# clysto/tinyimgcodec

Hardware: AMD Instinct MI355X
Metric: Mpixels/s encode (DCT+quant kernel) (higher is better)
Workload: dtype f32+f64

## Files before the change

tinyimgcodec_amd/csrc/tic_kernels.hip:

```cpp
#include <hip/hip_runtime.h>
#include <hip/hip_ext.h>
#include <stdint.h>
#include <stdlib.h>
#include <string.h>
#include <type_traits>

#include "tic_hooks.h"
#include "tic_kernels.h"
#include "tic_math.h"

namespace tic {

#define TIC_DPP_QP_XOR1 0xB1
#define TIC_DPP_QP_XOR2 0x4E
#define TIC_DPP_ROW_SHL4 0x104
#define TIC_DPP_ROW_SHR4 0x114

__device__ __forceinline__ uint32_t perm_b32(uint32_t hi_src, uint32_t lo_src, uint32_t sel) {
    return __builtin_amdgcn_perm(hi_src, lo_src, sel);
}

__device__ __forceinline__ void transpose8x8_bytes(uint32_t &lo, uint32_t &hi, int i) {
    uint32_t nhi = (uint32_t)__builtin_amdgcn_update_dpp((int)hi, (int)lo, TIC_DPP_ROW_SHL4, 0xf, 0x5, false);
    uint32_t nlo = (uint32_t)__builtin_amdgcn_update_dpp((int)lo, (int)hi, TIC_DPP_ROW_SHR4, 0xf, 0xa, false);
// ... 148 lines not shown
    const int lane = threadIdx.x & 63, wave = threadIdx.x >> 6;
    const int b = lane >> 3, i = lane & 7;
    uint32_t *lds = lds_all[wave];
    int tile = blockIdx.x * kWavesPerWG + wave;
    int ntiles = a.ntiles;
    if (a.rem_mode) {
        const int bh = a.ntiles / a.tiles_x, rw = a.tiles_x - a.fast_tx;
        const int n_right = bh * rw, n_bottom = (bh - a.fast_ty) * a.fast_tx;
        ntiles = 0;
        if (tile < n_right) {
            tile = (tile / rw) * a.tiles_x + a.fast_tx + tile % rw;
            ntiles = a.ntiles;
        } else if (tile < n_right + n_bottom) {
            const int k = tile - n_right;
            tile = (a.fast_ty + k / a.fast_tx) * a.tiles_x + k % a.fast_tx;
            ntiles = a.ntiles;
        }
    }
    Strip s = make_strip(tile, ntiles, a.tiles_x, a.bw, b);
    uint32_t lo, hi;
    load_block_row(a.img, a.h, a.w, a.stride, a.aligned8, s, i, lo, hi);
    transpose8x8_bytes(lo, hi, i);
    int q[8];
    exact_block(lo, hi, lds, b, i, a.consts, q);
    const uint4 zzv = *reinterpret_cast<const uint4 *>(a.consts->zzofs + i * 8);
    uint16_t zz[8] = {(uint16_t)zzv.x, (uint16_t)(zzv.x >> 16), (uint16_t)zzv.y, (uint16_t)(zzv.y >> 16),
                      (uint16_t)zzv.z, (uint16_t)(zzv.z >> 16), (uint16_t)zzv.w, (uint16_t)(zzv.w >> 16)};
    store_zigzag(lds, b, i, zz, q, a.out, s);
}

constexpr int kTWaveBytes = kLdsWaveBytes;
constexpr int kTHalfDw = 272;
constexpr int kZzWaveBytes = 8 * kZzStrideB;
constexpr int kPxBlkBytes = 80;
constexpr int kMaxStripsPerWave = 16;
constexpr int kChunkStrips = 8;

__device__ __forceinline__ void quant_fma(float z, float mul, uint32_t &bits, float &d) {
    const float s = fmaf(z, mul, kMagic);
    bits = __float_as_uint(s);
    const float nr = kMagic - s;
    d = fmaf(z, mul, nr);
}

__device__ __forceinline__ void store16_wt_nt(void *p, const uint4 &v) {
    typedef uint32_t u32x4 __attribute__((ext_vector_type(4)));
    const u32x4 d = {v.x, v.y, v.z, v.w};
    asm volatile("global_store_dwordx4 %0, %1, off sc1 nt" : : "v"(p), "v"(d) : "memory");
}
__device__ __forceinline__ void store16_wt_nt(const void *sbase, uint32_t voff, const uint4 &v) {
    typedef uint32_t u32x4 __attribute__((ext_vector_type(4)));
    const u32x4 d = {v.x, v.y, v.z, v.w};
    asm volatile("global_store_dwordx4 %0, %1, %2 sc1 nt" : : "v"(voff), "v"(d), "s"(sbase) : "memory");
}

constexpr int kMaxStripsPerWave2 = 64;
constexpr int kBatch = 8;
constexpr int kBatchWaveBytes = kBatch * (128 + 64) + 64;

template <int CTRL>
__device__ __forceinline__ double dpp_f64(double x) {
    const int lo = __builtin_amdgcn_mov_dpp(__double2loint(x), CTRL, 0xf, 0xf, true);
    const int hi = __builtin_amdgcn_mov_dpp(__double2hiint(x), CTRL, 0xf, 0xf, true);
    return __hiloint2double(hi, lo);
}

__device__ __forceinline__ int rational_quad(const uint32_t *ldsT, int b, int i, const double *cst_rat) {
#pragma clang fp contract(off)
    const int w = i >> 2, k = i & 3;
    const uint32_t ca = (0x05010300u >> (8 * k)) & 0xffu, cb = (0x06020407u >> (8 * k)) & 0xffu;
    const uint32_t *row = ldsT + w * 128 + 4 * b;
    const float fa = __uint_as_float(row[(ca >> 2) * kTHalfDw + (ca & 3)]);
    const float fb = __uint_as_float(row[(cb >> 2) * kTHalfDw + (cb & 3)]);
    const double K = w ? (kTW3 * 0.5) : (kSq2h * 0.5);
    const double ya = (double)fa * K, yb = (double)fb * K;
    const double p = ya + yb;
    const double s2 = p + dpp_f64<TIC_DPP_QP_XOR1>(p);
    const double o = dpp_f64<TIC_DPP_QP_XOR2>(s2);
    const double E = (k & 1) ? s2 - o : s2 + o;
    const double X = E * ((k & 1) ? (kTW3 * 0.5) : (kSq2h * 0.5));
    const double div = cst_rat[2 * w + (k & 1)], rdiv = cst_rat[4 + 2 * w + (k & 1)];
    return (int)rint(div_rn(X, div, rdiv));
}

__device__ __forceinline__ int rational_slim(uint32_t rowLo, uint32_t rowHi, int i, const double *cst_rat) {
#pragma clang fp contract(off)
    uint32_t lo = perm_b32(rowHi, rowLo, 0x04030700u);
    uint32_t hi = perm_b32(rowHi, rowLo, 0x06050201u);
    transpose8x8_bytes(lo, hi, i);
    const uint32_t tot = __builtin_amdgcn_sad_u8(lo, 0u, __builtin_amdgcn_sad_u8(hi, 0u, 0u));
    const uint32_t sa = __builtin_amdgcn_sad_u8(lo & 0xff0000ffu, 0u, __builtin_amdgcn_sad_u8(hi & 0xff0000ffu, 0u, 0u));
    const int e0 = (int)tot - 1024, e4 = 2 * (int)sa - (int)tot;
    double y0 = (double)e0 * (kSq2h * 0.5);
    double y4 = (double)e4 * (kTW3 * 0.5);
    y0 = y0 + dpp_f64<TIC_DPP_QP_XOR1>(y0);
    y4 = y4 + dpp_f64<TIC_DPP_QP_XOR1>(y4);
    y0 = y0 + dpp_f64<TIC_DPP_QP_XOR2>(y0);
    y4 = y4 + dpp_f64<TIC_DPP_QP_XOR2>(y4);
    const double b0 = dpp_f64<TIC_DPP_ROW_SHL4>(y0), b4 = dpp_f64<TIC_DPP_ROW_SHL4>(y4);
    const double A = (i & 2) ? y4 : y0, B = (i & 2) ? b4 : b0;
    const double E = (i & 1) ? A - B : A + B;
    const double X = E * ((i & 1) ? (kTW3 * 0.5) : (kSq2h * 0.5));
    const double div = cst_rat[i & 3], rdiv = cst_rat[4 + (i & 3)];
    return (int)rint(div_rn(X, div, rdiv));
}
__device__ __forceinline__ unsigned long long wave_redo_block(const uint8_t *px , double *tbuf ,
                                                              const double *cosm, const double *rdiv, const uint16_t *zzofs, int16_t *img16,
                                                              int lane) {
    const int u = lane >> 3, c = lane & 7;
    typedef double d2 __attribute__((ext_vector_type(2)));
    const d2 *mu = reinterpret_cast<const d2 *>(cosm + u * 8), *mc = reinterpret_cast<const d2 *>(cosm + c * 8);
    const d2 m0 = mu[0], m1 = mu[1], m2 = mu[2], m3 = mu[3];
    double x[8];
#pragma unroll
    for (int r = 0; r < 8; r++) x[r] = (double)((int)px[r * 8 + c] - 128);
    double ta = m0.x * x[0], tb = m0.y * x[1];
    ta = fma(m1.x, x[2], ta); tb = fma(m1.y, x[3], tb);
    ta = fma(m2.x, x[4], ta); tb = fma(m2.y, x[5], tb);
    ta = fma(m3.x, x[6], ta); tb = fma(m3.y, x[7], tb);
    tbuf[u * 8 + c] = ta + tb;
    const d2 n0 = mc[0], n1 = mc[1], n2 = mc[2], n3 = mc[3];
    wave_lds_fence();
    const d2 *tu = reinterpret_cast<const d2 *>(tbuf + u * 8);
    const d2 y0 = tu[0], y1 = tu[1], y2 = tu[2], y3 = tu[3];
    double xa = n0.x * y0.x, xb = n0.y * y0.y;
    xa = fma(n1.x, y1.x, xa); xb = fma(n1.y, y1.y, xb);
    xa = fma(n2.x, y2.x, xa); xb = fma(n2.y, y2.y, xb);
    xa = fma(n3.x, y3.x, xa); xb = fma(n3.y, y3.y, xb);
    const double X = xa + xb;
    const double tq = X * rdiv[lane], rq = rint(tq);
    const bool rational = (lane & 0x1b) == 0;
    const bool decided = fabs(tq - rq) < 0.5 - 1e-9;
    if (decided && !rational) img16[zzofs[lane] >> 1] = (int16_t)(int)rq;
    const unsigned long long und = __ballot(!decided && !rational);
    wave_lds_fence();
    return und;
}

__device__ __forceinline__ uint32_t second_level_8(uint32_t colLo, uint32_t colHi, uint32_t *lds, int b, int i, const double *mul64, int q[8]) {
    double c[8];
#pragma unroll
    for (int r = 0; r < 4; r++) {
        c[r] = (double)(int)((colLo >> (8 * r)) & 0xffu);
        c[r + 4] = (double)(int)((colHi >> (8 * r)) & 0xffu);
    }
    dct8_aan(c[0], c[1], c[2], c[3], c[4], c[5], c[6], c[7]);
    c[0] -= 1024.0;
    uint32_t w[8], wh[8];
#pragma unroll
    for (int k = 0; k < 8; k++) w[k] = (uint32_t)__double2loint(c[k]);
    transpose8x8_dwords(lds, b, i, w);
#pragma unroll
    for (int k = 0; k < 8; k++) wh[k] = (uint32_t)__double2hiint(c[k]);
    transpose8x8_dwords(lds, b, i, wh);
#pragma unroll
    for (int k = 0; k < 8; k++) c[k] = __hiloint2double((int)wh[k], (int)w[k]);
    dct8_aan(c[0], c[1], c[2], c[3], c[4], c[5], c[6], c[7]);
    uint32_t und = 0;
#pragma unroll
    for (int v = 0; v < 8; v++) {
        const double t = c[v] * mul64[i * 8 + v], r = rint(t);
        q[v] = (int)r;
        if (!(fabs(t - r) < 0.5 - 1e-9)) und |= 1u << v;
    }
    return und;
}

template <bool kCols>
__global__ __launch_bounds__(kWavesPerWG * 64, 6) __attribute__((amdgpu_num_vgpr(72))) void dctq_strip_kernel(DctqArgs a) {
    __shared__ __attribute__((aligned(16))) uint32_t ldsT_all[kWavesPerWG][kTWaveBytes / 4];
    __shared__ __attribute__((aligned(16))) uint32_t ldsZ_all[kWavesPerWG][kZzWaveBytes / 4];
    __shared__ __attribute__((aligned(16))) unsigned char cst_blk[kStripBlkBytes];
    __shared__ __attribute__((aligned(16))) uint32_t bat_all[kWavesPerWG][kBatchWaveBytes / 4];
    const int lane = threadIdx.x & 63;
    const int wave = __builtin_amdgcn_readfirstlane(threadIdx.x >> 6);
    uint32_t *ldsT = ldsT_all[wave];
    char *ldsZ = reinterpret_cast<char *>(ldsZ_all[wave]);
    const uint16_t *cst_zz = reinterpret_cast<const uint16_t *>(cst_blk + kBlkZz);
    const double *cst_rat = reinterpret_cast<const double *>(cst_blk + kBlkRat);
    uint4 *bat_img = reinterpret_cast<uint4 *>(bat_all[wave]);
    uint2 *bat_pix = reinterpret_cast<uint2 *>(bat_all[wave] + kBatch * 32);
    uint32_t *bat_id = bat_all[wave] + kBatch * 48;
    const DctqConsts *__restrict__ C = a.consts;
    a.img += (long)blockIdx.z * a.frame_stride_in;
    a.out = reinterpret_cast<int16_t *>(reinterpret_cast<char *>(a.out) + (long)blockIdx.z * a.frame_stride_out);

    const int lr = lane >> 3, lb = lane & 7;
    const int b = lane >> 3, i = lane & 7;
    unsigned long long mask_exact = 0;
    uint32_t n_second = 0, n_quad = 0;
    int nE = 0;
    int t_first, n_my;
    const uint32_t st_off = (uint32_t)lane * 16u;
    {
        typedef float f32x4 __attribute__((ext_vector_type(4)));
        typedef uint32_t u32x4 __attribute__((ext_vector_type(4)));
        f32x4 m0, m1;
        f32x4 thr;
        u32x4 zzv;
        u32x4 c_fill;
        {
            constexpr int kPpw = kStripBlkPieces / kWavesPerWG;
            static_assert(kPpw * kWavesPerWG == kStripBlkPieces && kPpw <= 64, "constant block must split evenly over the waves");
            const uint32_t piece = lane < kPpw ? (uint32_t)(wave * kPpw + lane) : (uint32_t)kStripBlkPieces - 1u;
            const uint32_t fo = piece * 16u;
            asm volatile("global_load_dwordx4 v[76:79], %0, %1" : : "v"(fo), "s"(C->strip_blk) : "memory", "v76", "v77", "v78", "v79");
        }
        const uint32_t px_wr = (uint32_t)(uintptr_t)(__attribute__((address_space(3))) char *)(ldsZ + lb * kPxBlkBytes + lr * 8);
        const uint8_t *px_rd = reinterpret_cast<const uint8_t *>(ldsZ + b * kPxBlkBytes + i);
        constexpr int kHalf = kCols ? kTHalfDw : 256;
        const int p1a = kCols ? i : lr, p1b = kCols ? b : lb;
        uint32_t *twA = ldsT + (p1a >> 2) * kHalf + (p1a & 3) + 4 * p1b;
        uint32_t *twB = ldsT + (p1a >> 2) * kHalf + (p1a & 3) + 4 * (p1b ^ 4);
        const uint4 *tr = reinterpret_cast<const uint4 *>(
            __builtin_assume_aligned(ldsT + i * 32 + 4 * (b ^ (4 * ((i >> 1) & 1))), 16));
        const uint32_t ld_off = (uint32_t)(lr * (int)a.stride + lb * 8);

        uint32_t tf, t_lim;
        if (a.team_count > 0) {
            const uint32_t r = blockIdx.y;
            const uint32_t row0 = (uint32_t)((r < 8u ? a.split_lo >> (8u * r) : a.split_hi) & 0xffull);
            const uint32_t row1 = (uint32_t)((r < 7u ? a.split_lo >> (8u * r + 8u) : a.split_hi) & 0xffull);
            tf = (row0 * (uint32_t)a.team_count + blockIdx.x) * kWavesPerWG + (uint32_t)wave;
            t_lim = tf + (row1 - row0) * (uint32_t)a.tstep;
        } else if (a.round_wgs > 0) {
            const uint32_t rho = a.magic_tstep ? __umulhi(blockIdx.x, a.magic_tstep ) : blockIdx.x;
            const uint32_t wl = blockIdx.x - rho * (uint32_t)a.round_wgs;
            const uint32_t base = rho * (uint32_t)a.round_wgs * (uint32_t)a.wg_span;
            tf = base + wl * kWavesPerWG + (uint32_t)wave;
            t_lim = base + (uint32_t)a.round_wgs * (uint32_t)a.wg_span;
        } else {
            tf = blockIdx.x * (uint32_t)a.wg_stride + (uint32_t)wave;
            t_lim = blockIdx.x * (uint32_t)a.wg_stride + (uint32_t)a.wg_span;
        }
        tf = __builtin_amdgcn_readfirstlane(tf);
        const uint32_t nfast = (uint32_t)a.fast_ty * (uint32_t)a.fast_tx;
        const uint32_t t_end = t_lim < nfast ? t_lim : nfast;
        n_my = 0;
        if (tf < t_end) n_my = (a.round_wgs > 0 || a.magic_tstep == 0u) ? (int)((t_end - tf + (uint32_t)a.tstep - 1u) / (uint32_t)a.tstep)
                                                                        : (int)__umulhi(t_end - tf + (uint32_t)a.tstep - 1u, a.magic_tstep);
        if (n_my == 0) tf = 0;
        t_first = (int)tf;
        const uint32_t ty_first = a.magic_fast_tx ? __umulhi(tf, a.magic_fast_tx) : tf;
        int txp = (int)(tf - ty_first * (uint32_t)a.fast_tx);
// ... 51 lines not shown
            float d0, d1, d2, d3, d4, d5, d6, d7;
            if constexpr (kCols) {
                d0 = (float)px_rd[0]; d1 = (float)px_rd[8]; d2 = (float)px_rd[16]; d3 = (float)px_rd[24];
                d4 = (float)px_rd[32]; d5 = (float)px_rd[40]; d6 = (float)px_rd[48]; d7 = (float)px_rd[56];
            } else {
                d0 = pxr[0]; d1 = pxr[1]; d2 = pxr[2]; d3 = pxr[3]; d4 = pxr[4]; d5 = pxr[5]; d6 = pxr[6]; d7 = pxr[7];
            }
            dct8_aan(d0, d1, d2, d3, d4, d5, d6, d7);
            d0 -= 1024.0f;
            twA[0 * 32] = __float_as_uint(d0); twA[1 * 32] = __float_as_uint(d1); twB[2 * 32] = __float_as_uint(d2);
            twB[3 * 32] = __float_as_uint(d3); twA[4 * 32] = __float_as_uint(d4); twA[5 * 32] = __float_as_uint(d5);
            twB[6 * 32] = __float_as_uint(d6); twB[7 * 32] = __float_as_uint(d7);
            wave_lds_fence();
            const uint4 ra = tr[0], rb = tr[kHalf / 4];
            wave_lds_fence();
            float e0 = __uint_as_float(ra.x), e1 = __uint_as_float(ra.y), e2 = __uint_as_float(ra.z), e3 = __uint_as_float(ra.w);
            float e4 = __uint_as_float(rb.x), e5 = __uint_as_float(rb.y), e6 = __uint_as_float(rb.z), e7 = __uint_as_float(rb.w);
            dct8_aan(e0, e1, e2, e3, e4, e5, e6, e7);
            uint32_t q0, q1, q2, q3, q4, q5, q6, q7;
            float r0, r1, r2, r3, r4, r5, r6, r7;
            quant_fma(e0, m0.x, q0, r0); quant_fma(e1, m0.y, q1, r1); quant_fma(e2, m0.z, q2, r2); quant_fma(e3, m0.w, q3, r3);
            quant_fma(e4, m1.x, q4, r4); quant_fma(e5, m1.y, q5, r5); quant_fma(e6, m1.z, q6, r6); quant_fma(e7, m1.w, q7, r7);
            const float mA1 = fmaxf(fmaxf(fabsf(r1), fabsf(r2)), fabsf(r3));
            const float mA2 = fmaxf(fmaxf(fabsf(r5), fabsf(r6)), fabsf(r7));
            const float mB = fmaxf(fabsf(r0), fabsf(r4));
            const unsigned long long cA = __ballot(mA1 > thr.x) | __ballot(mA2 > thr.y);
            const unsigned long long cB = __ballot(mB > thr.z);
            *zp0 = (int16_t)q0; *zp1 = (int16_t)q1; *zp2 = (int16_t)q2; *zp3 = (int16_t)q3;
            *zp4 = (int16_t)q4; *zp5 = (int16_t)q5; *zp6 = (int16_t)q6; *zp7 = (int16_t)q7;
            const unsigned long long kRat = 0x1111111111111111ull;
            if (__builtin_expect((cB & kRat) != 0ull, 0)) {
                n_quad++;
                if constexpr (kCols) {
                    const int rq = rational_quad(ldsT, b, i, cst_rat);
                    if ((i & 2) == 0) *zz_ptr(28u * (uint32_t)(i & 1) + 20u * (uint32_t)(i >> 2) + 30u * (uint32_t)((i & 1) & (i >> 2))) = (int16_t)rq;
                } else {
                    uint32_t lo0, hi0;
                    raw_words(tag, lo0, hi0);
                    uint2 *pb = reinterpret_cast<uint2 *>(ldsT);
                    pb[lb * 8 + lr] = make_uint2(lo0, hi0);
                    wave_lds_fence();
                    const uint2 rowv = pb[lane];
                    wave_lds_fence();
                    const int rq = rational_slim(rowv.x, rowv.y, i, cst_rat);
                    if (i < 4) *zz_ptr(i == 0 ? 0u : (i == 1 ? 28u : (i == 2 ? 20u : 78u))) = (int16_t)rq;
                }
            }
            wave_lds_fence();
            const uint4 val = *zr;
            wave_lds_fence();
            const char *dst = reinterpret_cast<const char *>(a.out) + ((unsigned long long)ob << 7);
            const unsigned long long mG = cA | (cB & ~kRat);
            if (__builtin_expect(mG != 0ull, 0)) {
                const uint32_t gm = (uint32_t)__ballot(((mG >> (8u * (uint32_t)i)) & 0xffull) != 0ull) & 0xffu;
                const int nnew = __builtin_popcount(gm);
                if (nE + nnew <= kBatch && gm != 0xffu) {
                    uint32_t lo0, hi0;
                    raw_words(tag, lo0, hi0);
                    const uint32_t below = (1u << b) - 1u, lbelow = (1u << lb) - 1u;
                    const bool mine = (gm >> b) & 1u;
                    const int e = nE + __builtin_popcount(gm & below);
                    if (mine) bat_img[e * 8 + i] = val;
                    if (mine && i == 0) bat_id[e] = ob + (uint32_t)b;
                    if ((gm >> lb) & 1u) bat_pix[(nE + __builtin_popcount(gm & lbelow)) * 8 + lr] = make_uint2(lo0, hi0);
                    if (!mine) store16_wt_nt(dst, st_off, val);
                    nE += nnew;
                    n_second += (uint32_t)nnew;
                } else {
                    mask_exact |= 1ull << kstrip;
                    store16_wt_nt(dst, st_off, val);
                }
            } else
                store16_wt_nt(dst, st_off, val);
            left--;
            kstrip++;
        };
        float pxf[8] = {0.f, 0.f, 0.f, 0.f, 0.f, 0.f, 0.f, 0.f};
#define TIC_STEP(RLOAD, OBL, RTAKE, R0, R1, OBP, N)                                                          \
        TIC_LOAD(RLOAD, OBL);                                                                                \
        if constexpr (kCols) { TIC_TAKE_COLS(RTAKE, N); } else { TIC_TAKE_ROWS(pxf, R0, R1, N); }            \
        process(std::integral_constant<int, R0>(), pxf, OBP)
        do {
            if (left == 0) break;
            TIC_STEP("76:77", ob2, "72:73", 72, 73, ob0, 2);
            if (left == 0) break;
            TIC_STEP("72:73", ob0, "74:75", 74, 75, ob1, 3);
            while (left != 0) {
                TIC_STEP("74:75", ob1, "76:77", 76, 77, ob2, 4);
                if (left == 0) break;
                TIC_STEP("76:77", ob2, "72:73", 72, 73, ob0, 4);
                if (left == 0) break;
                TIC_STEP("72:73", ob0, "74:75", 74, 75, ob1, 4);
            }
        } while (0);
#undef TIC_STEP
        asm volatile("; end of the strip walk" : : : TIC_RSV_CLOBBER);
#undef TIC_LOAD
#undef TIC_TAKE_COLS
#undef TIC_TAKE_ROWS
#undef TIC_RSV_CLOBBER
    }
    if (nE != 0) {
        const double *cst_cos = reinterpret_cast<const double *>(cst_blk + kBlkCos);
        const double *cst_rdiv = reinterpret_cast<const double *>(cst_blk + kBlkRdiv);
        uint32_t m_exact = 0;
        if (nE < 3) {
            for (int ee = 0; ee < nE; ee++) {
                const unsigned long long und = wave_redo_block(reinterpret_cast<const uint8_t *>(bat_pix + ee * 8), reinterpret_cast<double *>(ldsT), cst_cos,
                                                               cst_rdiv, cst_zz, reinterpret_cast<int16_t *>(bat_img + ee * 8), lane);
                if (und != 0ull) m_exact |= 1u << ee;
            }
        } else {
            const bool have2 = b < nE;
            const int e2 = have2 ? b : 0;
            const uint2 rowv = bat_pix[e2 * 8 + i];
            uint32_t lo = rowv.x, hi = rowv.y;
            transpose8x8_bytes(lo, hi, i);
            int qs[8];
            uint32_t und = second_level_8(lo, hi, ldsT, b, i, reinterpret_cast<const double *>(cst_blk + kBlkMul64), qs);
            if ((i & 3) == 0) und &= ~0x11u;
            const uint4 zo = *reinterpret_cast<const uint4 *>(cst_zz + i * 8);
            const uint32_t zw[4] = {zo.x, zo.y, zo.z, zo.w};
            int16_t *img2 = reinterpret_cast<int16_t *>(bat_img + e2 * 8);
            if (have2) {
#pragma unroll
                for (int v = 0; v < 8; v++)
                    if (!((und >> v) & 1u) && !((i & 3) == 0 && (v & 3) == 0)) img2[((zw[v >> 1] >> (16 * (v & 1))) & 0xffffu) >> 1] = (int16_t)qs[v];
            }
            const unsigned long long um = __ballot(have2 && und != 0u);
            for (int ee = 0; ee < nE; ee++)
                if ((um >> (8 * ee)) & 0xffull) m_exact |= 1u << ee;
        }
        const bool have = b < nE;
        const int e = have ? b : 0;
        const uint32_t blk = bat_id[e];
        if (m_exact != 0u) {
            const uint2 rowv = bat_pix[e * 8 + i];
            int16_t *img16 = reinterpret_cast<int16_t *>(bat_img + e * 8);
            uint32_t lo = rowv.x, hi = rowv.y;
            transpose8x8_bytes(lo, hi, i);
            const uint4 zo = *reinterpret_cast<const uint4 *>(cst_zz + i * 8);
            const uint32_t zw[4] = {zo.x, zo.y, zo.z, zo.w};
            int qx[8];
            exact_block(lo, hi, ldsT, b, i, C, qx);
            if (have && ((m_exact >> e) & 1u)) {
#pragma unroll
                for (int v = 0; v < 8; v++) img16[((zw[v >> 1] >> (16 * (v & 1))) & 0xffffu) >> 1] = (int16_t)qx[v];
            }
        }
        wave_lds_fence();
        const uint4 val = bat_img[e * 8 + i];
        if (have) store16_wt_nt(reinterpret_cast<char *>(a.out) + ((unsigned long long)blk << 7) + (uint32_t)i * 16u, val);
    }
    if (a.fallback_count != nullptr && lane == 0) {
        if (n_second != 0) atomicAdd(a.fallback_count, (unsigned long long)n_second);
        if (n_quad != 0) atomicAdd(a.fallback_count + 1, (unsigned long long)n_quad);
        if (mask_exact != 0ull) atomicAdd(a.fallback_count + 2, (unsigned long long)__builtin_popcountll(mask_exact));
        if (nE != 0) atomicMax(a.fallback_count + 3, (unsigned long long)nE);
    }
    if (mask_exact == 0ull) return;
    asm volatile("s_waitcnt vmcnt(0)" : : : "memory");
    const uint4 zzn = *reinterpret_cast<const uint4 *>(cst_zz + i * 8);
    const uint16_t zz[8] = {(uint16_t)zzn.x, (uint16_t)(zzn.x >> 16), (uint16_t)zzn.y, (uint16_t)(zzn.y >> 16),
                            (uint16_t)zzn.z, (uint16_t)(zzn.z >> 16), (uint16_t)zzn.w, (uint16_t)(zzn.w >> 16)};
    for (unsigned long long todo = mask_exact; todo != 0ull; todo &= todo - 1ull) {
        const int k = __builtin_ctzll(todo);
        const long t = (long)t_first + (long)k * a.tstep;
        const int ty = (int)(t / a.fast_tx), tx = (int)(t - (long)ty * a.fast_tx);
        Strip s;
        s.by = ty;
        s.bx = tx * 8 + b;
        s.valid = true;
        s.oblk = (size_t)ty * a.bw + s.bx;
        uint32_t lo, hi;
        load_block_row(a.img, a.h, a.w, a.stride, true, s, i, lo, hi);
        transpose8x8_bytes(lo, hi, i);
        int q[8];
        const uint32_t und = second_level_8(lo, hi, ldsT, b, i, reinterpret_cast<const double *>(cst_blk + kBlkMul64), q);
        if (__ballot(und != 0u) != 0ull) exact_block(lo, hi, ldsT, b, i, C, q);
        store_zigzag(reinterpret_cast<uint32_t *>(ldsZ), b, i, zz, q, a.out, s);
    }
}

__global__ __launch_bounds__(kWavesPerWG * 64) void dctq_exact_wide_kernel(WideArgs a) {
    __shared__ __attribute__((aligned(16))) uint32_t lds_all[kWavesPerWG][kLdsWaveBytes / 4];
    const int lane = threadIdx.x & 63, wave = threadIdx.x >> 6;
    const int b = lane >> 3, i = lane & 7;
    uint32_t *lds = lds_all[wave];
    const int tile = blockIdx.x * kWavesPerWG + wave;
    Strip s = make_strip(tile, a.ntiles, a.tiles_x, a.bw, b);
    double c[8];
#pragma unroll
    for (int r = 0; r < 8; r++) c[r] = 0.0;
    if (s.valid) {
        const int x = reflect_index(s.bx * 8 + i, a.w);
#pragma unroll
        for (int r = 0; r < 8; r++) {
            const int y = reflect_index(s.by * 8 + r, a.h);
            c[r] = (double)a.img[(long)y * a.stride + x] - 128.0;
        }
    }
    dct8_exact(c[0], c[1], c[2], c[3], c[4], c[5], c[6], c[7]);
    uint32_t w[8], wh[8];
#pragma unroll
    for (int k = 0; k < 8; k++) w[k] = (uint32_t)__double2loint(c[k]);
    transpose8x8_dwords(lds, b, i, w);
#pragma unroll
    for (int k = 0; k < 8; k++) wh[k] = (uint32_t)__double2hiint(c[k]);
    transpose8x8_dwords(lds, b, i, wh);
#pragma unroll
    for (int k = 0; k < 8; k++) c[k] = __hiloint2double((int)wh[k], (int)w[k]);
    dct8_exact(c[0], c[1], c[2], c[3], c[4], c[5], c[6], c[7]);
    if (!s.valid) return;
    const double *div = a.consts->div + i * 8;
    const uint16_t *zz = a.consts->zzofs + i * 8;
    int32_t *ob = a.out + s.oblk * 64;
#pragma unroll
    for (int v = 0; v < 8; v++) {
        ob[zz[v] >> 1] = (int32_t)rint(c[v] / div[v]);
        __builtin_amdgcn_sched_barrier(0);
    }
}

__constant__ int kAnnScalesInt[64] = {
    16384, 22725, 21407, 19266, 16384, 12873, 8867,  4520,  22725, 31521, 29692, 26722, 22725, 17855, 12299, 6270,
    21407, 29692, 27969, 25172, 21407, 16819, 11585, 5906,  19266, 26722, 25172, 22654, 19266, 15137, 10426, 5315,
    16384, 22725, 21407, 19266, 16384, 12873, 8867,  4520,  12873, 17855, 16819, 15137, 12873, 10114, 6967,  3552,
    8867,  12299, 11585, 10426, 8867,  6967,  4799,  2446,  4520,  6270,  5906,  5315,  4520,  3552,  2446,  1247};

__global__ __launch_bounds__(kWavesPerWG * 64) void idct_kernel(IdctArgs a) {
    __shared__ __attribute__((aligned(16))) uint32_t lds_all[kWavesPerWG][kLdsWaveBytes / 4];
    const int lane = threadIdx.x & 63, wave = threadIdx.x >> 6;
    const int b = lane >> 3, i = lane & 7;
// ... 278 lines not shown
```

tinyimgcodec_amd/csrc/tic_math.h:

```cpp
#pragma once
#include <math.h>
#include <stdint.h>
#include <string.h>

#include "tic_tables.h"

#if defined(__HIPCC__)
#define TIC_HD __host__ __device__ __forceinline__
#else
#define TIC_HD inline
#endif

namespace tic {

TIC_HD void dct8_exact(double &c0, double &c1, double &c2, double &c3, double &c4, double &c5, double &c6,
                       double &c7) {
#pragma clang fp contract(off)
    c0 = c0 * 2.0;
    c7 = c7 * 2.0;
    double t;
    t = c2; c2 = t - c1; c1 = t + c1;
    t = c4; c4 = t - c3; c3 = t + c3;
    t = c6; c6 = t - c5; c5 = t + c5;
    double h0 = c0 + c7, h4 = c0 - c7;
// ... 54 lines not shown
    t = c5; c5 = t - c6; c6 = t + c6;
}
TIC_HD void idct8_exact(double &c0, double &c1, double &c2, double &c3, double &c4, double &c5, double &c6, double &c7) {
    idct8_exact_impl<true>(c0, c1, c2, c3, c4, c5, c6, c7);
}

TIC_HD double div_rn(double a, double b, double y ) {
    const double q0 = a * y;
    const double r0 = fma(-q0, b, a);
    const double q1 = fma(r0, y, q0);
    const double r1 = fma(-q1, b, a);
    return fma(r1, y, q1);
}

TIC_HD float tic_fma(float a, float b, float c) { return fmaf(a, b, c); }
TIC_HD double tic_fma(double a, double b, double c) { return fma(a, b, c); }

template <typename T>
TIC_HD void dct8_aan(T &d0, T &d1, T &d2, T &d3, T &d4, T &d5, T &d6, T &d7) {
#pragma clang fp contract(off)
    const T c707 = (T)0.70710678118654752440, c382 = (T)0.38268343236508977173;
    const T c541 = (T)0.54119610014619698440, c1306 = (T)1.30656296487637652786;
    T t0 = d0 + d7, t7 = d0 - d7, t1 = d1 + d6, t6 = d1 - d6;
    T t2 = d2 + d5, t5 = d2 - d5, t3 = d3 + d4, t4 = d3 - d4;
    T t10 = t0 + t3, t13 = t0 - t3, t11 = t1 + t2, t12 = t1 - t2;
    d0 = t10 + t11;
    d4 = t10 - t11;
    T s = t12 + t13;
    d2 = tic_fma(s, c707, t13);
    d6 = tic_fma(s, -c707, t13);
    T u10 = t4 + t5, u11 = t5 + t6, u12 = t6 + t7;
    T z5 = (u10 - u12) * c382;
    T z2 = tic_fma(u10, c541, z5);
    T z4 = tic_fma(u12, c1306, z5);
    T z11 = tic_fma(u11, c707, t7);
    T z13 = tic_fma(u11, -c707, t7);
    d5 = z13 + z2;
    d3 = z13 - z2;
    d1 = z11 + z4;
    d7 = z11 - z4;
}

static constexpr double kGuard[64] = {
    6.2256e-05, 3.2315e-04, 2.6249e-04, 3.4557e-04, 6.2256e-05, 3.3290e-04, 2.0056e-04, 5.9516e-04,
    1.8850e-04, 3.9880e-04, 3.3279e-04, 4.4030e-04, 1.8850e-04, 4.2003e-04, 2.8730e-04, 7.1855e-04,
    1.1955e-04, 3.1685e-04, 2.7439e-04, 3.5239e-04, 1.1955e-04, 3.3094e-04, 2.2674e-04, 5.9192e-04,
    1.8674e-04, 3.7822e-04, 3.2467e-04, 4.1881e-04, 1.8674e-04, 3.9724e-04, 2.9065e-04, 6.9278e-04,
    6.2256e-05, 3.2315e-04, 2.6249e-04, 3.4557e-04, 6.2256e-05, 3.3290e-04, 2.0056e-04, 5.9516e-04,
    2.1405e-04, 4.9996e-04, 4.2070e-04, 5.6244e-04, 2.1405e-04, 5.6214e-04, 3.5821e-04, 9.0797e-04,
    1.1428e-04, 6.1485e-04, 5.1255e-04, 7.0510e-04, 1.1428e-04, 6.6162e-04, 3.4923e-04, 1.0793e-03,
    5.1054e-04, 1.5901e-03, 1.3262e-03, 1.8402e-03, 5.1054e-04, 1.7563e-03, 1.0117e-03, 2.7581e-03,
};
constexpr double guard_cf(int u, int v) { return kGuard[v * 8 + u]; }
static constexpr float kMagic = 12582912.0f;

struct DctqConsts {
    double div[64];
    double rdiv[64];
    float mulN[64];
    double mul64[64];
    float mulT[64];
    float thrG[32];
    uint16_t zzofsT[64];
    float thrR[32];
    double cosm[64];
    uint16_t zzofs[64];
    uint8_t zznat[64];
    alignas(16) unsigned char strip_blk[2624];
};
constexpr int kStripBlkBytes = 2624;
constexpr int kStripBlkPieces = kStripBlkBytes / 16;
constexpr int kBlkMul = 0, kBlkThr = 256, kBlkZz = 384, kBlkRat = 512, kBlkCos = 576, kBlkRdiv = 1088, kBlkMul64 = 1600;
constexpr int kBlkMulT = 2112, kBlkThrT = 2368, kBlkZzT = 2496;

inline float thr_below(double tau) {
    float f = (float)tau;
    if ((double)f > tau) f = nextafterf(f, 0.0f);
    return nextafterf(f, 0.0f);
}

inline bool build_consts(double quality, DctqConsts *c) {
#pragma clang fp contract(off)
    if (!(quality >= 1.0 && quality <= 99.0)) return false;
    const double factor = quality < 50.0 ? 5000.0 / quality : 200.0 - 2.0 * quality;
    for (int i = 0; i < 64; i++) {
        const double p = (double)kQTable[i] * factor;
        c->div[i] = p / 100.0;
        c->rdiv[i] = 1.0 / c->div[i];
    }
    double aan[8];
    aan[0] = 1.0;
    for (int k = 1; k < 8; k++) aan[k] = sqrt(2.0) * cos(k * 3.14159265358979323846 / 16.0);
    for (int u = 0; u < 8; u++)
        for (int v = 0; v < 8; v++) {
            c->mul64[u * 8 + v] = 1.0 / (aan[u] * aan[v] * 8.0 * c->div[u * 8 + v]);
            c->mulN[u * 8 + v] = (float)c->mul64[u * 8 + v];
        }
    for (int u = 0; u < 8; u++)
        for (int v = 0; v < 8; v++) c->mulT[v * 8 + u] = c->mulN[u * 8 + v];
    for (int v = 0; v < 8; v++) {
        double g3[3] = {0.0, 0.0, 0.0};
        for (int u = 0; u < 8; u++) {
            const double g = kGuard[u * 8 + v] / c->div[u * 8 + v];
            const int grp = (u == 0 || u == 4) ? 2 : (u < 4 ? 0 : 1);
            if (g > g3[grp]) g3[grp] = g;
        }
        for (int k = 0; k < 3; k++) c->thrG[4 * v + k] = thr_below(0.5 - g3[k]);
        c->thrG[4 * v + 3] = 0.0f;
    }
    for (int u = 0; u < 8; u++) {
        double g3[3] = {0.0, 0.0, 0.0};
        for (int v = 0; v < 8; v++) {
            const double g = guard_cf(u, v) / c->div[u * 8 + v];
            const int grp = (v == 0 || v == 4) ? 2 : (v < 4 ? 0 : 1);
            if (g > g3[grp]) g3[grp] = g;
        }
        for (int k = 0; k < 3; k++) c->thrR[4 * u + k] = thr_below(0.5 - g3[k]);
        c->thrR[4 * u + 3] = 0.0f;
    }
    for (int k = 0; k < 8; k++)
        for (int n = 0; n < 8; n++)
            c->cosm[k * 8 + n] = (k == 0 ? sqrt(0.125) : 0.5) * cos((2 * n + 1) * k * 3.14159265358979323846 / 16.0);
    for (int k = 0; k < 64; k++) {
        int nat = kZigzag[k];
        c->zzofs[nat] = (uint16_t)(2 * k);
        c->zzofsT[(nat & 7) * 8 + (nat >> 3)] = (uint16_t)(2 * k);
        c->zznat[k] = (uint8_t)nat;
    }
    {
        unsigned char *p = c->strip_blk;
        memset(p, 0, kStripBlkBytes);
        memcpy(p + kBlkMul, c->mulN, 256);
        memcpy(p + kBlkThr, c->thrR, 128);
        memcpy(p + kBlkZz, c->zzofs, 128);
        const int rat[4] = {0, 4, 32, 36};
        for (int k = 0; k < 4; k++) {
            memcpy(p + kBlkRat + 8 * k, &c->div[rat[k]], 8);
            memcpy(p + kBlkRat + 32 + 8 * k, &c->rdiv[rat[k]], 8);
        }
        memcpy(p + kBlkCos, c->cosm, 512);
        memcpy(p + kBlkRdiv, c->rdiv, 512);
        memcpy(p + kBlkMul64, c->mul64, 512);
        memcpy(p + kBlkMulT, c->mulT, 256);
        memcpy(p + kBlkThrT, c->thrG, 128);
        memcpy(p + kBlkZzT, c->zzofsT, 128);
    }
    return true;
}
inline bool build_consts(int quality, DctqConsts *c) { return build_consts((double)quality, c); }


}
```

Measured before the change: 1.838 million.

## Add magnitude-aware refined guard test to skip exact fallback for blocks

When the coarse guard flags a block as possibly misrounded, a second test now recomputes the float AAN DCT and quantization residual and compares it against a threshold that scales with the block's and row's maximum input magnitude. Only blocks that still fail this test go to the batched exact (f64) path, and blocks that pass are stored directly. This is meant to cut the number of expensive exact recomputations. In exchange the flagged path does extra float DCT work, DPP reductions and constant loads, and the constant block grows to hold the new per-coefficient tables.

```diff
diff --git a/tinyimgcodec_amd/csrc/tic_kernels.hip b/tinyimgcodec_amd/csrc/tic_kernels.hip
--- a/tinyimgcodec_amd/csrc/tic_kernels.hip
+++ b/tinyimgcodec_amd/csrc/tic_kernels.hip
@@ -224,6 +224,15 @@
     typedef uint32_t u32x4 __attribute__((ext_vector_type(4)));
     const u32x4 d = {v.x, v.y, v.z, v.w};
     asm volatile("global_store_dwordx4 %0, %1, %2 sc1 nt" : : "v"(voff), "v"(d), "s"(sbase) : "memory");
+}
+
+__device__ __forceinline__ float max_over_block(float m) {
+    m = fmaxf(m, __int_as_float(__builtin_amdgcn_mov_dpp(__float_as_int(m), TIC_DPP_QP_XOR1, 0xf, 0xf, true)));
+    m = fmaxf(m, __int_as_float(__builtin_amdgcn_mov_dpp(__float_as_int(m), TIC_DPP_QP_XOR2, 0xf, 0xf, true)));
+    const int mi = __float_as_int(m);
+    int o = __builtin_amdgcn_update_dpp(mi, mi, TIC_DPP_ROW_SHL4, 0xf, 0x5, false);
+    o = __builtin_amdgcn_update_dpp(o, mi, TIC_DPP_ROW_SHR4, 0xf, 0xa, false);
+    return fmaxf(m, __int_as_float(o));
 }
 
 constexpr int kMaxStripsPerWave2 = 64;
@@ -519,9 +528,38 @@
             const char *dst = reinterpret_cast<const char *>(a.out) + ((unsigned long long)ob << 7);
             const unsigned long long mG = cA | (cB & ~kRat);
             if (__builtin_expect(mG != 0ull, 0)) {
-                const uint32_t gm = (uint32_t)__ballot(((mG >> (8u * (uint32_t)i)) & 0xffull) != 0ull) & 0xffu;
+                unsigned long long mR = mG;
+                if (kCols || (cB & kRat) == 0ull) {
+                    uint32_t so = st_off;
+                    asm volatile("" : "+v"(so));
+                    const uint32_t ln = so >> 4, li = ln & 7u;
+                    const uint4 sa = tr[0], sb = tr[kHalf / 4];
+                    float f[8] = {__uint_as_float(sa.x), __uint_as_float(sa.y), __uint_as_float(sa.z), __uint_as_float(sa.w),
+                                  __uint_as_float(sb.x), __uint_as_float(sb.y), __uint_as_float(sb.z), __uint_as_float(sb.w)};
+                    const float Mv = fmaxf(fmaxf(fmaxf(fmaxf(fabsf(f[0]), fabsf(f[1])), fabsf(f[2])), fmaxf(fmaxf(fabsf(f[3]), fabsf(f[4])), fabsf(f[5]))),
+                                           fmaxf(fabsf(f[6]), fabsf(f[7])));
+                    const float Mb = max_over_block(Mv);
+                    dct8_aan(f[0], f[1], f[2], f[3], f[4], f[5], f[6], f[7]);
+                    __builtin_amdgcn_sched_barrier(0);
+                    const float *rc = reinterpret_cast<const float *>(cst_blk + (kCols ? kBlkRefC : kBlkRefCT) + li * 32u);
+                    const uint32_t *rw = reinterpret_cast<const uint32_t *>(cst_blk + (kCols ? kBlkRefB : kBlkRefBT) + li * 32u);
+                    const float mm[8] = {m0.x, m0.y, m0.z, m0.w, m1.x, m1.y, m1.z, m1.w};
+                    bool inside = false;
+#pragma unroll
+                    for (int v = 0; v < 8; v++) {
+                        uint32_t qb;
+                        float dd;
+                        quant_fma(f[v], mm[v], qb, dd);
+                        inside |= refined_trip(fabsf(dd), rc[v], rw[v], Mb, Mv);
+                        __builtin_amdgcn_sched_barrier(0);
+                    }
+                    mR = __ballot(inside && ((mG >> ln) & 1ull) != 0ull);
+                }
+                const uint32_t gm = (uint32_t)__ballot(((mR >> (8u * (uint32_t)i)) & 0xffull) != 0ull) & 0xffu;
                 const int nnew = __builtin_popcount(gm);
-                if (nE + nnew <= kBatch && gm != 0xffu) {
+                if (gm == 0u) {
+                    store16_wt_nt(dst, st_off, val);
+                } else if (nE + nnew <= kBatch && gm != 0xffu) {
                     uint32_t lo0, hi0;
                     raw_words(tag, lo0, hi0);
                     const uint32_t below = (1u << b) - 1u, lbelow = (1u << lb) - 1u;
diff --git a/tinyimgcodec_amd/csrc/tic_math.h b/tinyimgcodec_amd/csrc/tic_math.h
--- a/tinyimgcodec_amd/csrc/tic_math.h
+++ b/tinyimgcodec_amd/csrc/tic_math.h
@@ -130,6 +130,39 @@
     5.1054e-04, 1.5901e-03, 1.3262e-03, 1.8402e-03, 5.1054e-04, 1.7563e-03, 1.0117e-03, 2.7581e-03,
 };
 constexpr double guard_cf(int u, int v) { return kGuard[v * 8 + u]; }
+static constexpr double kGuardA[64] = {
+    1.3518e-12, 2.5249e-05, 9.6364e-06, 5.3537e-06, 1.0619e-12, 1.3123e-05, 2.3265e-05, 1.3802e-04,
+    2.5249e-05, 3.3960e-05, 1.9711e-05, 2.1118e-05, 2.5249e-05, 2.5005e-05, 2.7011e-05, 1.2867e-04,
+    9.6364e-06, 1.9711e-05, 1.7806e-05, 1.3067e-05, 9.6364e-06, 1.5604e-05, 2.5182e-05, 1.3246e-04,
+    5.3537e-06, 2.1118e-05, 1.3067e-05, 8.7636e-06, 5.3537e-06, 1.3371e-05, 2.2877e-05, 1.2748e-04,
+    1.0619e-12, 2.5249e-05, 9.6364e-06, 5.3537e-06, 1.0619e-12, 1.3123e-05, 2.3265e-05, 1.3802e-04,
+    1.3123e-05, 2.5005e-05, 1.5604e-05, 1.3371e-05, 1.3123e-05, 1.8564e-05, 2.4978e-05, 1.2875e-04,
+    2.3265e-05, 2.7011e-05, 2.5182e-05, 2.2877e-05, 2.3265e-05, 2.4978e-05, 3.0397e-05, 1.3625e-04,
+    1.3802e-04, 1.2867e-04, 1.3246e-04, 1.2748e-04, 1.3802e-04, 1.2875e-04, 1.3625e-04, 2.2213e-04,
+};
+static constexpr double kGuardB1[64] = {
+    0.0000e+00, 1.6250e-07, 4.6532e-08, 1.9168e-07, 0.0000e+00, 2.8686e-07, 1.1234e-07, 8.1691e-07,
+    0.0000e+00, 1.9208e-07, 5.5002e-08, 2.2657e-07, 0.0000e+00, 3.3908e-07, 1.3279e-07, 9.6561e-07,
+    0.0000e+00, 1.5013e-07, 4.2990e-08, 1.7709e-07, 0.0000e+00, 2.6503e-07, 1.0379e-07, 7.5473e-07,
+    0.0000e+00, 1.7369e-07, 4.9736e-08, 2.0487e-07, 0.0000e+00, 3.0661e-07, 1.2008e-07, 8.7315e-07,
+    0.0000e+00, 1.6250e-07, 4.6532e-08, 1.9168e-07, 0.0000e+00, 2.8686e-07, 1.1234e-07, 8.1691e-07,
+    0.0000e+00, 2.5994e-07, 7.4435e-08, 3.0661e-07, 0.0000e+00, 4.5888e-07, 1.7971e-07, 1.3068e-06,
+    0.0000e+00, 3.6243e-07, 1.0379e-07, 4.2752e-07, 0.0000e+00, 6.3983e-07, 2.5057e-07, 1.8221e-06,
+    0.0000e+00, 9.6561e-07, 2.7652e-07, 1.1391e-06, 0.0000e+00, 1.7047e-06, 6.6757e-07, 4.8545e-06,
+};
+static constexpr double kGuardB2[64] = {
+    6.0797e-08, 1.7533e-07, 1.8613e-07, 2.0682e-07, 6.0797e-08, 3.0952e-07, 4.4936e-07, 8.8144e-07,
+    1.8205e-07, 2.3906e-07, 2.5379e-07, 2.8199e-07, 1.8205e-07, 4.2203e-07, 6.1269e-07, 1.2019e-06,
+    1.1234e-07, 1.8571e-07, 1.9715e-07, 2.1906e-07, 1.1234e-07, 3.2784e-07, 4.7595e-07, 9.3360e-07,
+    1.9495e-07, 2.3920e-07, 2.5393e-07, 2.8215e-07, 1.9495e-07, 4.2227e-07, 6.1304e-07, 1.2026e-06,
+    6.0797e-08, 1.7533e-07, 1.8613e-07, 2.0682e-07, 6.0797e-08, 3.0952e-07, 4.4936e-07, 8.8144e-07,
+    2.3705e-07, 3.1854e-07, 3.3816e-07, 3.7574e-07, 2.3705e-07, 5.6233e-07, 8.1638e-07, 1.6014e-06,
+    1.1234e-07, 3.3379e-07, 3.5435e-07, 3.9374e-07, 1.1234e-07, 5.8927e-07, 8.5548e-07, 1.6781e-06,
+    4.7147e-07, 8.8193e-07, 9.3625e-07, 1.0403e-06, 4.7147e-07, 1.5570e-06, 2.2603e-06, 4.4338e-06,
+};
+constexpr double guard_a_cf(int u, int v) { return kGuardA[v * 8 + u]; }
+constexpr double guard_b1_cf(int u, int v) { return kGuardB1[v * 8 + u]; }
+constexpr double guard_b2_cf(int u, int v) { return kGuardB2[v * 8 + u]; }
 static constexpr float kMagic = 12582912.0f;
 
 struct DctqConsts {
@@ -144,17 +177,42 @@
     double cosm[64];
     uint16_t zzofs[64];
     uint8_t zznat[64];
-    alignas(16) unsigned char strip_blk[2624];
-};
-constexpr int kStripBlkBytes = 2624;
+    float refC[64];
+    uint32_t refB[64];
+    float refCT[64];
+    uint32_t refBT[64];
+    alignas(16) unsigned char strip_blk[3648];
+};
+constexpr int kStripBlkBytes = 3648;
 constexpr int kStripBlkPieces = kStripBlkBytes / 16;
 constexpr int kBlkMul = 0, kBlkThr = 256, kBlkZz = 384, kBlkRat = 512, kBlkCos = 576, kBlkRdiv = 1088, kBlkMul64 = 1600;
 constexpr int kBlkMulT = 2112, kBlkThrT = 2368, kBlkZzT = 2496;
+constexpr int kBlkRefC = 2624, kBlkRefB = 2880, kBlkRefCT = 3136, kBlkRefBT = 3392;
 
 inline float thr_below(double tau) {
     float f = (float)tau;
     if ((double)f > tau) f = nextafterf(f, 0.0f);
     return nextafterf(f, 0.0f);
+}
+
+inline float thr_refined(double tau) { return nextafterf(thr_below(tau), 0.0f); }
+inline uint32_t ref_b_up(double x) {
+    float f = (float)x;
+    if ((double)f < x) f = nextafterf(f, 1.0f);
+    uint32_t w;
+    memcpy(&w, &f, 4);
+    return (w + 0xffffu) >> 16;
+}
+TIC_HD float ref_bits(uint32_t b) {
+    float f;
+    memcpy(&f, &b, 4);
+    return f;
+}
+TIC_HD float ref_b1(uint32_t w) { return ref_bits(w & 0xffff0000u); }
+TIC_HD float ref_b2(uint32_t w) { return ref_bits(w << 16); }
+TIC_HD bool refined_trip(float dabs, float c, uint32_t w, float Mb, float Mv) {
+    const float thr = fmaf(-ref_b1(w), Mb, fmaf(-ref_b2(w), Mv, c));
+    return dabs > thr;
 }
 
 inline bool build_consts(double quality, DctqConsts *c) {
@@ -196,6 +254,15 @@
         for (int k = 0; k < 3; k++) c->thrR[4 * u + k] = thr_below(0.5 - g3[k]);
         c->thrR[4 * u + 3] = 0.0f;
     }
+    for (int u = 0; u < 8; u++)
+        for (int v = 0; v < 8; v++) {
+            const bool rational = (u & 3) == 0 && (v & 3) == 0;
+            const double d = c->div[u * 8 + v];
+            c->refC[u * 8 + v] = rational ? 1.0f : thr_refined(0.5 - guard_a_cf(u, v) / d);
+            c->refB[u * 8 + v] = rational ? 0u : (ref_b_up(guard_b1_cf(u, v) / d) << 16) | ref_b_up(guard_b2_cf(u, v) / d);
+            c->refCT[v * 8 + u] = rational ? 1.0f : thr_refined(0.5 - kGuardA[u * 8 + v] / d);
+            c->refBT[v * 8 + u] = rational ? 0u : (ref_b_up(kGuardB1[u * 8 + v] / d) << 16) | ref_b_up(kGuardB2[u * 8 + v] / d);
+        }
     for (int k = 0; k < 8; k++)
         for (int n = 0; n < 8; n++)
             c->cosm[k * 8 + n] = (k == 0 ? sqrt(0.125) : 0.5) * cos((2 * n + 1) * k * 3.14159265358979323846 / 16.0);
@@ -222,6 +289,10 @@
         memcpy(p + kBlkMulT, c->mulT, 256);
         memcpy(p + kBlkThrT, c->thrG, 128);
         memcpy(p + kBlkZzT, c->zzofsT, 128);
+        memcpy(p + kBlkRefC, c->refC, 256);
+        memcpy(p + kBlkRefB, c->refB, 256);
+        memcpy(p + kBlkRefCT, c->refCT, 256);
+        memcpy(p + kBlkRefBT, c->refBT, 256);
     }
     return true;
 }
```

Result: slower. 1.659 million (-9.7%).

## Replace LDS batch buffer with deferred re-fetch and per-strip redo of tripped blocks

Applied to the files above, without the earlier changes.

Strips whose fast path trips the ambiguity check no longer stash pixels and quantized rows in a per-wave LDS batch area during the main loop. Every strip is stored immediately and only records a compact per-strip block mask. Afterwards each tripped strip reloads its pixels from global memory, recomputes the rational and second-level or exact results in the zigzag LDS scratch, and rewrites only the affected blocks. This removes the batch LDS allocation and bookkeeping from the hot loop, which should lower LDS pressure and allow more occupancy. In exchange, rare strips are written twice and their pixels reloaded, and the tile index division now uses a magic multiply.

```diff
diff --git a/tinyimgcodec_amd/csrc/tic_kernels.hip b/tinyimgcodec_amd/csrc/tic_kernels.hip
--- a/tinyimgcodec_amd/csrc/tic_kernels.hip
+++ b/tinyimgcodec_amd/csrc/tic_kernels.hip
@@ -227,8 +227,8 @@
 }
 
 constexpr int kMaxStripsPerWave2 = 64;
+constexpr int kTripMasks = 8;
 constexpr int kBatch = 8;
-constexpr int kBatchWaveBytes = kBatch * (128 + 64) + 64;
 
 template <int CTRL>
 __device__ __forceinline__ double dpp_f64(double x) {
@@ -291,8 +291,8 @@
     ta = fma(m2.x, x[4], ta); tb = fma(m2.y, x[5], tb);
     ta = fma(m3.x, x[6], ta); tb = fma(m3.y, x[7], tb);
     tbuf[u * 8 + c] = ta + tb;
+    wave_lds_fence();
     const d2 n0 = mc[0], n1 = mc[1], n2 = mc[2], n3 = mc[3];
-    wave_lds_fence();
     const d2 *tu = reinterpret_cast<const d2 *>(tbuf + u * 8);
     const d2 y0 = tu[0], y1 = tu[1], y2 = tu[2], y3 = tu[3];
     double xa = n0.x * y0.x, xb = n0.y * y0.y;
@@ -343,25 +343,22 @@
     __shared__ __attribute__((aligned(16))) uint32_t ldsT_all[kWavesPerWG][kTWaveBytes / 4];
     __shared__ __attribute__((aligned(16))) uint32_t ldsZ_all[kWavesPerWG][kZzWaveBytes / 4];
     __shared__ __attribute__((aligned(16))) unsigned char cst_blk[kStripBlkBytes];
-    __shared__ __attribute__((aligned(16))) uint32_t bat_all[kWavesPerWG][kBatchWaveBytes / 4];
     const int lane = threadIdx.x & 63;
     const int wave = __builtin_amdgcn_readfirstlane(threadIdx.x >> 6);
     uint32_t *ldsT = ldsT_all[wave];
     char *ldsZ = reinterpret_cast<char *>(ldsZ_all[wave]);
     const uint16_t *cst_zz = reinterpret_cast<const uint16_t *>(cst_blk + kBlkZz);
     const double *cst_rat = reinterpret_cast<const double *>(cst_blk + kBlkRat);
-    uint4 *bat_img = reinterpret_cast<uint4 *>(bat_all[wave]);
-    uint2 *bat_pix = reinterpret_cast<uint2 *>(bat_all[wave] + kBatch * 32);
-    uint32_t *bat_id = bat_all[wave] + kBatch * 48;
     const DctqConsts *__restrict__ C = a.consts;
     a.img += (long)blockIdx.z * a.frame_stride_in;
     a.out = reinterpret_cast<int16_t *>(reinterpret_cast<char *>(a.out) + (long)blockIdx.z * a.frame_stride_out);
 
     const int lr = lane >> 3, lb = lane & 7;
     const int b = lane >> 3, i = lane & 7;
-    unsigned long long mask_exact = 0;
-    uint32_t n_second = 0, n_quad = 0;
-    int nE = 0;
+    unsigned long long mask_trip = 0;
+    unsigned long long trip_gm = 0;
+    int n_trip = 0;
+    uint32_t n_quad = 0;
     int t_first, n_my;
     const uint32_t st_off = (uint32_t)lane * 16u;
     {
@@ -520,25 +517,11 @@
             const unsigned long long mG = cA | (cB & ~kRat);
             if (__builtin_expect(mG != 0ull, 0)) {
                 const uint32_t gm = (uint32_t)__ballot(((mG >> (8u * (uint32_t)i)) & 0xffull) != 0ull) & 0xffu;
-                const int nnew = __builtin_popcount(gm);
-                if (nE + nnew <= kBatch && gm != 0xffu) {
-                    uint32_t lo0, hi0;
-                    raw_words(tag, lo0, hi0);
-                    const uint32_t below = (1u << b) - 1u, lbelow = (1u << lb) - 1u;
-                    const bool mine = (gm >> b) & 1u;
-                    const int e = nE + __builtin_popcount(gm & below);
-                    if (mine) bat_img[e * 8 + i] = val;
-                    if (mine && i == 0) bat_id[e] = ob + (uint32_t)b;
-                    if ((gm >> lb) & 1u) bat_pix[(nE + __builtin_popcount(gm & lbelow)) * 8 + lr] = make_uint2(lo0, hi0);
-                    if (!mine) store16_wt_nt(dst, st_off, val);
-                    nE += nnew;
-                    n_second += (uint32_t)nnew;
-                } else {
-                    mask_exact |= 1ull << kstrip;
-                    store16_wt_nt(dst, st_off, val);
-                }
-            } else
-                store16_wt_nt(dst, st_off, val);
+                if (n_trip < kTripMasks) trip_gm |= (unsigned long long)gm << (8 * n_trip);
+                n_trip++;
+                mask_trip |= 1ull << kstrip;
+            }
+            store16_wt_nt(dst, st_off, val);
             left--;
             kstrip++;
         };
@@ -567,85 +550,95 @@
 #undef TIC_TAKE_ROWS
 #undef TIC_RSV_CLOBBER
     }
-    if (nE != 0) {
+    uint32_t n_second = 0, n_whole = 0;
+    int nE = 0;
+    if (mask_trip != 0ull) {
         const double *cst_cos = reinterpret_cast<const double *>(cst_blk + kBlkCos);
         const double *cst_rdiv = reinterpret_cast<const double *>(cst_blk + kBlkRdiv);
-        uint32_t m_exact = 0;
-        if (nE < 3) {
-            for (int ee = 0; ee < nE; ee++) {
-                const unsigned long long und = wave_redo_block(reinterpret_cast<const uint8_t *>(bat_pix + ee * 8), reinterpret_cast<double *>(ldsT), cst_cos,
-                                                               cst_rdiv, cst_zz, reinterpret_cast<int16_t *>(bat_img + ee * 8), lane);
-                if (und != 0ull) m_exact |= 1u << ee;
-            }
-        } else {
-            const bool have2 = b < nE;
-            const int e2 = have2 ? b : 0;
-            const uint2 rowv = bat_pix[e2 * 8 + i];
-            uint32_t lo = rowv.x, hi = rowv.y;
+        const double *cst_mul64 = reinterpret_cast<const double *>(cst_blk + kBlkMul64);
+        int lane2 = (int)__builtin_amdgcn_mbcnt_hi(~0u, __builtin_amdgcn_mbcnt_lo(~0u, 0u));
+        int rec = 0;
+        for (unsigned long long todo = mask_trip; todo != 0ull; todo &= todo - 1ull, rec++) {
+            const int k = __builtin_ctzll(todo);
+            const uint32_t gm = rec < kTripMasks ? (uint32_t)(trip_gm >> (8 * rec)) & 0xffu : 0xffu;
+            const int nnew = __builtin_popcount(gm);
+            const uint32_t t = (uint32_t)t_first + (uint32_t)k * (uint32_t)a.tstep;
+            const uint32_t uty = a.magic_fast_tx ? __umulhi(t, a.magic_fast_tx) : t;
+            const int ty = (int)uty, tx = (int)(t - uty * (uint32_t)a.fast_tx);
+            const bool whole = gm == 0xffu || nE + nnew > kBatch;
+            if (whole) {
+                n_whole++;
+            } else {
+                nE += nnew;
+                n_second += (uint32_t)nnew;
+            }
+            asm volatile("" : "+v"(lane2));
+            const int b = lane2 >> 3, i = lane2 & 7;
+            const bool mine = whole || ((gm >> b) & 1u);
+            auto put_row = [&](const int (&qv)[8], uint32_t skip) {
+                const uint4 zo = *reinterpret_cast<const uint4 *>(cst_zz + i * 8);
+                const uint32_t zw[4] = {zo.x, zo.y, zo.z, zo.w};
+                int16_t *img = reinterpret_cast<int16_t *>(ldsZ + b * 128);
+#pragma unroll
+                for (int v = 0; v < 8; v++)
+                    if (!((skip >> v) & 1u)) img[((zw[v >> 1] >> (16 * (v & 1))) & 0xffffu) >> 1] = (int16_t)qv[v];
+            };
+            Strip s;
+            s.by = ty;
+            s.bx = tx * 8 + b;
+            s.valid = true;
+            s.oblk = (size_t)ty * a.bw + s.bx;
+            uint32_t lo, hi;
+            load_block_row(a.img, a.h, a.w, a.stride, true, s, i, lo, hi);
+            asm volatile("s_waitcnt vmcnt(0)" : : : "memory");
+            const int rq = rational_slim(lo, hi, i, cst_rat);
+            if (i < 4) reinterpret_cast<int16_t *>(ldsZ + b * 128)[i == 0 ? 0 : (i == 1 ? 14 : (i == 2 ? 10 : 39))] = (int16_t)rq;
+            uint32_t m_exact = 0;
+            if (!whole && nnew < 3) {
+                uint2 *pix = reinterpret_cast<uint2 *>(ldsT + 128);
+                pix[lane2] = make_uint2(lo, hi);
+                wave_lds_fence();
+                for (uint32_t gg = gm; gg != 0u; gg &= gg - 1u) {
+                    const int bb = __builtin_ctz(gg);
+                    int lane3 = lane2;
+                    asm volatile("" : "+v"(lane3));
+                    const unsigned long long und = wave_redo_block(reinterpret_cast<const uint8_t *>(pix + bb * 8), reinterpret_cast<double *>(ldsT), cst_cos,
+                                                                   cst_rdiv, cst_zz, reinterpret_cast<int16_t *>(ldsZ + bb * 128), lane3);
+                    if (und != 0ull) m_exact |= 1u << bb;
+                }
+                const uint2 pv = pix[lane2];
+                lo = pv.x;
+                hi = pv.y;
+                wave_lds_fence();
+            }
             transpose8x8_bytes(lo, hi, i);
-            int qs[8];
-            uint32_t und = second_level_8(lo, hi, ldsT, b, i, reinterpret_cast<const double *>(cst_blk + kBlkMul64), qs);
-            if ((i & 3) == 0) und &= ~0x11u;
-            const uint4 zo = *reinterpret_cast<const uint4 *>(cst_zz + i * 8);
-            const uint32_t zw[4] = {zo.x, zo.y, zo.z, zo.w};
-            int16_t *img2 = reinterpret_cast<int16_t *>(bat_img + e2 * 8);
-            if (have2) {
-#pragma unroll
-                for (int v = 0; v < 8; v++)
-                    if (!((und >> v) & 1u) && !((i & 3) == 0 && (v & 3) == 0)) img2[((zw[v >> 1] >> (16 * (v & 1))) & 0xffffu) >> 1] = (int16_t)qs[v];
-            }
-            const unsigned long long um = __ballot(have2 && und != 0u);
-            for (int ee = 0; ee < nE; ee++)
-                if ((um >> (8 * ee)) & 0xffull) m_exact |= 1u << ee;
-        }
-        const bool have = b < nE;
-        const int e = have ? b : 0;
-        const uint32_t blk = bat_id[e];
-        if (m_exact != 0u) {
-            const uint2 rowv = bat_pix[e * 8 + i];
-            int16_t *img16 = reinterpret_cast<int16_t *>(bat_img + e * 8);
-            uint32_t lo = rowv.x, hi = rowv.y;
-            transpose8x8_bytes(lo, hi, i);
-            const uint4 zo = *reinterpret_cast<const uint4 *>(cst_zz + i * 8);
-            const uint32_t zw[4] = {zo.x, zo.y, zo.z, zo.w};
-            int qx[8];
-            exact_block(lo, hi, ldsT, b, i, C, qx);
-            if (have && ((m_exact >> e) & 1u)) {
-#pragma unroll
-                for (int v = 0; v < 8; v++) img16[((zw[v >> 1] >> (16 * (v & 1))) & 0xffffu) >> 1] = (int16_t)qx[v];
-            }
-        }
-        wave_lds_fence();
-        const uint4 val = bat_img[e * 8 + i];
-        if (have) store16_wt_nt(reinterpret_cast<char *>(a.out) + ((unsigned long long)blk << 7) + (uint32_t)i * 16u, val);
+            if (whole || nnew >= 3) {
+                int qs[8];
+                uint32_t und = second_level_8(lo, hi, ldsT, b, i, cst_mul64, qs);
+                if ((i & 3) == 0) und &= ~0x11u;
+                put_row(qs, und | ((i & 3) == 0 ? 0x11u : 0u));
+                const unsigned long long um = __ballot(mine && und != 0u);
+                for (int bb = 0; bb < 8; bb++)
+                    if ((um >> (8 * bb)) & 0xffull) m_exact |= 1u << bb;
+            }
+            if (m_exact != 0u) {
+                wave_lds_fence();
+                int qx[8];
+                exact_block(lo, hi, ldsT, b, i, C, qx);
+                if ((m_exact >> b) & 1u) put_row(qx, 0u);
+            }
+            wave_lds_fence();
+            const uint4 val = *reinterpret_cast<const uint4 *>(ldsZ + b * 128 + i * 16);
+            wave_lds_fence();
+            const char *dst = reinterpret_cast<const char *>(a.out) + (((unsigned long long)uty * (unsigned long long)a.bw + (unsigned long long)tx * 8ull) << 7);
+            if (mine) store16_wt_nt(dst, (uint32_t)lane2 * 16u, val);
+        }
     }
     if (a.fallback_count != nullptr && lane == 0) {
         if (n_second != 0) atomicAdd(a.fallback_count, (unsigned long long)n_second);
         if (n_quad != 0) atomicAdd(a.fallback_count + 1, (unsigned long long)n_quad);
-        if (mask_exact != 0ull) atomicAdd(a.fallback_count + 2, (unsigned long long)__builtin_popcountll(mask_exact));
+        if (n_whole != 0) atomicAdd(a.fallback_count + 2, (unsigned long long)n_whole);
         if (nE != 0) atomicMax(a.fallback_count + 3, (unsigned long long)nE);
-    }
-    if (mask_exact == 0ull) return;
-    asm volatile("s_waitcnt vmcnt(0)" : : : "memory");
-    const uint4 zzn = *reinterpret_cast<const uint4 *>(cst_zz + i * 8);
-    const uint16_t zz[8] = {(uint16_t)zzn.x, (uint16_t)(zzn.x >> 16), (uint16_t)zzn.y, (uint16_t)(zzn.y >> 16),
-                            (uint16_t)zzn.z, (uint16_t)(zzn.z >> 16), (uint16_t)zzn.w, (uint16_t)(zzn.w >> 16)};
-    for (unsigned long long todo = mask_exact; todo != 0ull; todo &= todo - 1ull) {
-        const int k = __builtin_ctzll(todo);
-        const long t = (long)t_first + (long)k * a.tstep;
-        const int ty = (int)(t / a.fast_tx), tx = (int)(t - (long)ty * a.fast_tx);
-        Strip s;
-        s.by = ty;
-        s.bx = tx * 8 + b;
-        s.valid = true;
-        s.oblk = (size_t)ty * a.bw + s.bx;
-        uint32_t lo, hi;
-        load_block_row(a.img, a.h, a.w, a.stride, true, s, i, lo, hi);
-        transpose8x8_bytes(lo, hi, i);
-        int q[8];
-        const uint32_t und = second_level_8(lo, hi, ldsT, b, i, reinterpret_cast<const double *>(cst_blk + kBlkMul64), q);
-        if (__ballot(und != 0u) != 0ull) exact_block(lo, hi, ldsT, b, i, C, q);
-        store_zigzag(reinterpret_cast<uint32_t *>(ldsZ), b, i, zz, q, a.out, s);
     }
 }
 
```

Result: slower. 1.683 million before, 1.570 million after (-6.8%).
